# matteospanio/torchfx

Measured on AMD Instinct MI355X. Metric: Msamples/s/GPU (64-ch fused biquad→FIR→FFT-conv chain); % HBM roofline, higher is better.
Workload: dtype f64 (IIR) + f32 (FFT); f32 I/O

## Files before the change

### torchfx_amd/csrc/ols_kernels.h

```cpp
#pragma once
#include "common.h"
#include "epilogue.h"
#include "fftpk.h"

namespace tfx {

typedef float2 cpx;

__device__ __forceinline__ cpx cmul(cpx a, cpx b) { return make_float2(a.x * b.x - a.y * b.y, a.x * b.y + a.y * b.x); }
__device__ __forceinline__ cpx cmulc(cpx a, cpx b) { return make_float2(a.x * b.x + a.y * b.y, a.y * b.x - a.x * b.y); }
__device__ __forceinline__ cpx cadd(cpx a, cpx b) { return make_float2(a.x + b.x, a.y + b.y); }
__device__ __forceinline__ cpx csub(cpx a, cpx b) { return make_float2(a.x - b.x, a.y - b.y); }

template <bool INV>
__device__ __forceinline__ void dft4(cpx &a0, cpx &a1, cpx &a2, cpx &a3)
{
    const cpx s02 = cadd(a0, a2), d02 = csub(a0, a2), s13 = cadd(a1, a3), d13 = csub(a1, a3);
    const cpx id = INV ? make_float2(-d13.y, d13.x) : make_float2(d13.y, -d13.x);
    a0 = cadd(s02, s13);
    a2 = csub(s02, s13);
    a1 = cadd(d02, id);
    a3 = csub(d02, id);
}

__device__ __forceinline__ void wave_sync2()
{
    __builtin_amdgcn_fence(__ATOMIC_RELEASE, "wavefront");
    __builtin_amdgcn_wave_barrier();
    __builtin_amdgcn_fence(__ATOMIC_ACQUIRE, "wavefront");
}

struct OlsGeom {
    int64_t Tn;
    int64_t Tout;
    int64_t F;
    int64_t S;
    int64_t t0;
    int64_t pad_left;
    int64_t out_shift;
    int64_t nframes;
    const float *hist;
    int64_t H;
    float ep_gain;
    int ep_scale, ep_clamp, ep_stat;
    double *ep_partial;
    int64_t ep_row;
    int N2;
    int P2;
    int sh_on, sh_base;
    int *nf_flag;
    int *nf_pair;
    int nt;
};

constexpr int OLS_N1 = 256;
constexpr int OLS_CB = 32;

__device__ __forceinline__ int pad16(int p) { return p + (p >> 4); }
__device__ __forceinline__ int row_shift(const OlsGeom &g, int64_t c) { return g.sh_on ? (int)(((int64_t)g.sh_base + c * g.Tn) & 31) : 0; }


template <bool INV, int NBF, bool LEAN = false>
__device__ __forceinline__ void col_stages16(cpx (&v)[NBF][16], cpx *lds, const cpx *tw256, int col, int q)
{
    constexpr int QS = 16 / NBF;
    using pk::v2f;
    const v2f Wc = {0.92387953251128675613f, 0.38268343236508977173f}, Wr = {0.70710678118654752440f, 0.70710678118654752440f};
    v2f *L = (v2f *)lds;
    const v2f *TW = (const v2f *)tw256;
#pragma unroll
    for (int i = 0; i < NBF; ++i) {
        v2f u[16];
#pragma unroll
        for (int t = 0; t < 16; ++t) u[t] = __builtin_bit_cast(v2f, v[i][t]);
        pk::pk_dft16<INV>(u, Wc, Wr);
        const int j = q + QS * i;
#pragma unroll
        for (int k = 0; k < 16; ++k) L[(16 * j + k) * OLS_CB + col] = u[PK_DFT16_AT(k)];
    }
    __syncthreads();
#pragma unroll
    for (int i = 0; i < NBF; ++i) {
        const int j = q + QS * i;
        v2f d[16], w[16];
#pragma unroll
        for (int t = 0; t < 16; ++t) d[t] = L[(j + 16 * t) * OLS_CB + col];
        if (LEAN) {
#pragma unroll
            for (int b = 0; b < 4; ++b) {
#pragma unroll
                for (int t = 0; t < 4; ++t) if (4 * b + t > 0) w[t] = TW[((4 * b + t) * j) & 255];
                __builtin_amdgcn_sched_barrier(0);
#pragma unroll
                for (int t = 0; t < 4; ++t) if (4 * b + t > 0) d[4 * b + t] = pk::pk_cmul<INV>(d[4 * b + t], w[t]);
            }
        } else {
#pragma unroll
            for (int t = 1; t < 16; ++t) w[t] = TW[(t * j) & 255];
            __builtin_amdgcn_sched_barrier(0);
#pragma unroll
            for (int t = 1; t < 16; ++t) d[t] = pk::pk_cmul<INV>(d[t], w[t]);
        }
        pk::pk_dft16<INV>(d, Wc, Wr);
#pragma unroll
        for (int t = 0; t < 16; ++t) v[i][t] = __builtin_bit_cast(cpx, d[t]);
    }
}

template <int NBF>
__global__ void __launch_bounds__(512 / NBF, 2)
ols_col_fwd16_kernel(const float *__restrict__ x, cpx *__restrict__ T, const cpx *__restrict__ tw256g,
                     OlsGeom g, int64_t frame0)
{
    constexpr int QS = 16 / NBF;
    extern __shared__ __attribute__((aligned(16))) char smem[];
    cpx *lds = (cpx *)smem;
    cpx *tw256 = lds + OLS_N1 * OLS_CB;
    const int tid = threadIdx.x, col = tid & 31, q = tid >> 5;
    if (tid < 256) tw256[tid] = tw256g[tid];
    const int ncb = g.N2 / OLS_CB;
    const int64_t pair = blockIdx.x / ncb;
    const int cb = blockIdx.x % ncb;
    const int n2 = cb * OLS_CB + col;
    const int64_t fa = frame0 + 2 * pair, fb = fa + 1;
    const int64_t ca = fa / g.F, ia0 = g.t0 + (fa % g.F) * g.S - g.pad_left - row_shift(g, ca);
    const bool has_b = fb < g.nframes;
    const int64_t cb_ = has_b ? fb / g.F : 0, ib0 = has_b ? g.t0 + (fb % g.F) * g.S - g.pad_left - row_shift(g, cb_) : 0;
    const float *xa = x + ca * g.Tn, *xb = x + cb_ * g.Tn;
    cpx v[NBF][16];
    const int64_t span = (int64_t)OLS_N1 * g.N2;
    const bool inner = ia0 >= 0 && ia0 + span <= g.Tn && has_b && ib0 >= 0 && ib0 + span <= g.Tn;
    if (inner && (g.nt & 1)) {
#pragma unroll
        for (int i = 0; i < NBF; ++i)
#pragma unroll
            for (int t = 0; t < 16; ++t) {
                const int64_t n = (int64_t)(q + QS * i + 16 * t) * g.N2 + n2;
                v[i][t] = make_float2(__builtin_nontemporal_load(xa + ia0 + n), __builtin_nontemporal_load(xb + ib0 + n));
            }
    } else if (inner) {
#pragma unroll
        for (int i = 0; i < NBF; ++i)
#pragma unroll
            for (int t = 0; t < 16; ++t) {
                const int64_t n = (int64_t)(q + QS * i + 16 * t) * g.N2 + n2;
                v[i][t] = make_float2(xa[ia0 + n], xb[ib0 + n]);
            }
    } else {
#pragma unroll
        for (int i = 0; i < NBF; ++i)
#pragma unroll
            for (int t = 0; t < 16; ++t) {
                const int64_t n = (int64_t)(q + QS * i + 16 * t) * g.N2 + n2;
                const int64_t ia = ia0 + n, ib = ib0 + n;
                float re = (ia >= 0 && ia < g.Tn) ? xa[ia] : 0.0f;
                float im = (has_b && ib >= 0 && ib < g.Tn) ? xb[ib] : 0.0f;
                if (g.hist) {
                    if (ia < 0 && ia >= -g.H) re = g.hist[ca * g.H + g.H + ia];
                    if (has_b && ib < 0 && ib >= -g.H) im = g.hist[cb_ * g.H + g.H + ib];
                }
                v[i][t] = make_float2(re, im);
            }
    }
    if (has_b && ca != cb_ && g.nf_pair) {
        bool bad_a = false, bad_b = false;
#pragma unroll
        for (int i = 0; i < NBF; ++i)
#pragma unroll
            for (int t = 0; t < 16; ++t) {
                if (!(__builtin_fabsf(v[i][t].x) <= 3.4028234663852886e38f)) { v[i][t].x = 0.0f; bad_a = true; }
                if (!(__builtin_fabsf(v[i][t].y) <= 3.4028234663852886e38f)) { v[i][t].y = 0.0f; bad_b = true; }
            }
        if (bad_a) atomicOr(&g.nf_pair[ca], 2);
        if (bad_b) atomicOr(&g.nf_pair[cb_], 1);
    }
    __syncthreads();
    col_stages16<false, NBF>(v, lds, tw256, col, q);
    cpx *Tp = T + pair * ((int64_t)OLS_N1 * g.P2);
#pragma unroll
    for (int i = 0; i < NBF; ++i)
#pragma unroll
        for (int k = 0; k < 16; ++k)
            Tp[(int64_t)(q + QS * i + 16 * k) * g.P2 + n2] = v[i][PK_DFT16_AT(k)];
}

template <int NBF>
__global__ void __launch_bounds__(512 / NBF, 2)
ols_col_inv16_kernel(const cpx *__restrict__ T, float *__restrict__ y, const cpx *__restrict__ tw256g,
                     OlsGeom g, int64_t frame0)
{
    constexpr int QS = 16 / NBF;
    extern __shared__ __attribute__((aligned(16))) char smem[];
    cpx *lds = (cpx *)smem;
    cpx *tw256 = lds + OLS_N1 * OLS_CB;
    const int tid = threadIdx.x, col = tid & 31, q = tid >> 5;
    if (tid < 256) tw256[tid] = tw256g[tid];
    const int ncb = g.N2 / OLS_CB;
    const int64_t pair = blockIdx.x / ncb;
    const int cb = blockIdx.x % ncb;
    const int n2 = cb * OLS_CB + col;
    const cpx *Tp = T + pair * ((int64_t)OLS_N1 * g.P2);
    cpx v[NBF][16];
#pragma unroll
    for (int i = 0; i < NBF; ++i)
#pragma unroll
        for (int t = 0; t < 16; ++t) v[i][t] = Tp[(int64_t)(q + QS * i + 16 * t) * g.P2 + n2];
    __syncthreads();
    col_stages16<true, NBF>(v, lds, tw256, col, q);

    const int64_t fa = frame0 + 2 * pair, fb = fa + 1;
    const int64_t ca = fa / g.F, oa0 = g.t0 + (fa % g.F) * g.S;
    const bool has_b = fb < g.nframes;
    const int64_t cb_ = has_b ? fb / g.F : 0, ob0 = has_b ? g.t0 + (fb % g.F) * g.S : 0;
    float *ya = y + ca * g.Tout, *yb = y + cb_ * g.Tout;
    const int64_t sha = g.out_shift + row_shift(g, ca), shb = g.out_shift + row_shift(g, cb_);
    const bool epi = g.ep_scale | g.ep_clamp | (g.ep_stat >= 0);
    double acc_a = 0.0, acc_b = 0.0;
#pragma unroll
    for (int i = 0; i < NBF; ++i)
#pragma unroll
        for (int k = 0; k < 16; ++k) {
            const int64_t n = (int64_t)(q + QS * i + 16 * k) * g.N2 + n2;
            if (n < g.S) {
                cpx o = v[i][PK_DFT16_AT(k)];
                const int64_t oa = oa0 + n - sha, ob = ob0 + n - shb;
                const bool wa = oa >= 0 && oa < g.Tout, wb = has_b && ob >= 0 && ob < g.Tout;
                if (epi) {
                    if (g.ep_scale) { o.x *= g.ep_gain; o.y *= g.ep_gain; }
                    if (g.ep_clamp) { o.x = clamp_unit(o.x); o.y = clamp_unit(o.y); }
                    if (g.ep_stat >= 0) {
                        if (wa) acc_a = red_comb_rt(g.ep_stat, acc_a, red_elem_rt(g.ep_stat, (double)o.x));
                        if (wb) acc_b = red_comb_rt(g.ep_stat, acc_b, red_elem_rt(g.ep_stat, (double)o.y));
                    }
                }
                if (g.nt & 2) {
                    if (wa) __builtin_nontemporal_store(o.x, ya + oa);
                    if (wb) __builtin_nontemporal_store(o.y, yb + ob);
                } else {
                    if (wa) ya[oa] = o.x;
                    if (wb) yb[ob] = o.y;
                }
            }
        }
    if (g.ep_stat >= 0) {
        double *red = (double *)smem;
        __syncthreads();
#pragma unroll
        for (int off = 32; off >= 1; off >>= 1) {
            acc_a = red_comb_rt(g.ep_stat, acc_a, __shfl_xor(acc_a, off));
            acc_b = red_comb_rt(g.ep_stat, acc_b, __shfl_xor(acc_b, off));
        }
        const int nw = (int)(blockDim.x >> 6), w = tid >> 6;
        if ((tid & 63) == 0) { red[w] = acc_a; red[nw + w] = acc_b; }
        __syncthreads();
        if (tid == 0) {
            double ra = red[0], rb = red[nw];
            for (int u = 1; u < nw; ++u) { ra = red_comb_rt(g.ep_stat, ra, red[u]); rb = red_comb_rt(g.ep_stat, rb, red[nw + u]); }
            g.ep_partial[ca * g.ep_row + (fa % g.F) * ncb + cb] = ra;
            if (has_b) g.ep_partial[cb_ * g.ep_row + (fb % g.F) * ncb + cb] = rb;
        }
    }
}

__global__ void __launch_bounds__(256) ols_straddle_fix_kernel(float *__restrict__ y, OlsGeom g)
{
    const int64_t c = blockIdx.x;
    const int flag = g.nf_pair[c];
    if (!flag) return;
    const int64_t org = g.t0 - g.out_shift - row_shift(g, c);
    for (int e = 0; e < 2; ++e) {
        if (!(flag & (1 << e))) continue;
        const int64_t f = e ? g.F - 1 : 0;
        if (blockIdx.y == 0 && threadIdx.x == 0 && g.ep_stat >= 0) g.ep_partial[c * g.ep_row + f * (g.N2 / OLS_CB)] = __builtin_nan("");
        const int64_t lo = max((int64_t)0, org + f * g.S), hi = min(g.Tout, org + (f + 1) * g.S);
        for (int64_t t = lo + (int64_t)blockIdx.y * 256 + threadIdx.x; t < hi; t += (int64_t)gridDim.y * 256) y[c * g.Tout + t] = __builtin_nanf("");
    }
}

constexpr int SOSF_MAXK = 8;
constexpr int SOSF_K4W = 4;
constexpr int SOSF_CH = 16;
constexpr int SOSF_LS = 36;
constexpr size_t OLS_SHM_SOSF = (size_t)512 * SOSF_LS * sizeof(float) + 256 * sizeof(cpx);
struct SosFuse {
    double co[SOSF_MAXK][5];
    double *sections;
    int warm_blocks;
    int prio;
};

template <int KS, bool TAPS, bool UNIT>
__global__ void __launch_bounds__(512, ((KS <= SOSF_K4W && !TAPS) ? 4 : 2))
ols_col_fwd16_sos_kernel(const float *__restrict__ x, cpx *__restrict__ T, const cpx *__restrict__ tw256g,
                         OlsGeom g, int64_t frame0, SosFuse sf)
{
    extern __shared__ __attribute__((aligned(16))) char smem[];
    float *S = (float *)smem;
    cpx *lds = (cpx *)smem;
    cpx *tw256 = (cpx *)(smem + (size_t)512 * SOSF_LS * sizeof(float));
    const int tid = threadIdx.x;
    if (tid < 256) tw256[tid] = tw256g[tid];
    const int64_t pair = blockIdx.x;
    const int64_t fa = frame0 + 2 * pair, fb = fa + 1;
    const int64_t ca = fa / g.F, ia0 = g.t0 + (fa % g.F) * g.S - g.pad_left - row_shift(g, ca);
    const bool has_b = fb < g.nframes;
    const int64_t cb_ = has_b ? fb / g.F : 0, ib0 = has_b ? g.t0 + (fb % g.F) * g.S - g.pad_left - row_shift(g, cb_) : 0;
    const float *xa = x + ca * g.Tn, *xb = x + cb_ * g.Tn;
    const int nblk = g.N2 / OLS_CB;
    int64_t ta = ia0 - (int64_t)OLS_CB * sf.warm_blocks, tb = ib0 - (int64_t)OLS_CB * sf.warm_blocks;
    auto bound = [](int64_t v) { return (int)(v < -(int64_t)0x40000000 ? -(int64_t)0x40000000 : (v > (int64_t)0x40000000 ? (int64_t)0x40000000 : v)); };

    const bool mine_b = tid >= 256;
    const int rel_l = (tid & 255) * g.N2;
    const int own_lo = TAPS ? ((((mine_b ? fb : fa) % g.F) == 0 && g.t0 == 0) ? 0 : OLS_N1 * g.N2 - (int)g.S) : 0;
    double h1[KS + 1], h2[KS + 1];
#pragma unroll
    for (int s = 0; s <= KS; ++s) { h1[s] = 0.0; h2[s] = 0.0; }

    const int lrow = tid >> 3, lpart = tid & 7;
    const int rel_f = lrow * g.N2 + 4 * lpart;
    const int rstep = 64 * g.N2;
    float4 P[8];
    auto fetch = [&]() {
        const float *pa = xa + ta, *pb = xb + tb;
        const int lo_a = bound(-ta), hi_a = bound(g.Tn - ta), lo_b = bound(-tb), hi_b = has_b ? bound(g.Tn - tb) : lo_b;
        int rel = rel_f;
        asm volatile("" : "+v"(rel));
#pragma unroll
        for (int i = 0; i < 8; ++i) {
            const bool isb = i >= 4;
            const int r = rel + (i & 3) * rstep;
            const int lo = isb ? lo_b : lo_a, hi = isb ? hi_b : hi_a;
            float4 v = make_float4(0.f, 0.f, 0.f, 0.f);
            if (r >= lo && r + 4 <= hi) {
                const float *src = (isb ? pb : pa) + r;
                v = (g.nt & 1) ? ldg16_stream<float4>(src) : *(const float4 *)src;
            } else if (r + 4 > lo && r < hi) {
                const float *src = (isb ? pb : pa) + r;
                if (r >= lo) v.x = src[0];
                if (r + 1 >= lo && r + 1 < hi) v.y = src[1];
                if (r + 2 >= lo && r + 2 < hi) v.z = src[2];
                if (r + 3 < hi) v.w = src[3];
            }
            P[i] = v;
        }
        ta += OLS_CB; tb += OLS_CB;
    };
    fetch();
    cpx *Tp = T + pair * ((int64_t)OLS_N1 * g.P2);
    const int col = tid & 31, q = tid >> 5;
    for (int blk = -sf.warm_blocks; blk < nblk; ++blk) {
#pragma unroll
        for (int i = 0; i < 8; ++i) *(float4 *)&S[(lrow + 64 * i) * SOSF_LS + 4 * lpart] = P[i];
        int64_t tcur = (mine_b ? tb : ta) - OLS_CB;
        {
            const unsigned lo32 = (unsigned)__builtin_amdgcn_readfirstlane((int)(unsigned)(uint64_t)tcur);
            const unsigned hi32 = (unsigned)__builtin_amdgcn_readfirstlane((int)(unsigned)((uint64_t)tcur >> 32));
            tcur = (int64_t)(((uint64_t)hi32 << 32) | lo32);
        }
        const int last = (!mine_b || has_b) ? min(max(bound(g.Tn - tcur) - rel_l, 0), OLS_CB) : 0;
        int first = 0;
        if (TAPS) first = max(min(max(bound(-tcur) - rel_l, 0), OLS_CB), min(max(own_lo - (rel_l + OLS_CB * blk), 0), OLS_CB));
        if (blk + 1 < nblk) fetch();
        __syncthreads();
        if (sf.prio) __builtin_amdgcn_s_setprio(0);
#pragma unroll 1
        for (int j = 0; j < OLS_CB / SOSF_CH; ++j) {
            float u[SOSF_CH];
#pragma unroll
            for (int i = 0; i < SOSF_CH / 4; ++i) {
                const float4 w4 = *(const float4 *)&S[tid * SOSF_LS + SOSF_CH * j + 4 * i];
                u[4 * i] = w4.x; u[4 * i + 1] = w4.y; u[4 * i + 2] = w4.z; u[4 * i + 3] = w4.w;
            }
            const int lastj = last - SOSF_CH * j, firstj = first - SOSF_CH * j;
#pragma unroll
            for (int n = 0; n < SOSF_CH; ++n) {
                double v = (double)u[n];
#pragma unroll
                for (int s = 0; s < KS; ++s) {
                    double yn = UNIT ? __builtin_fma(sf.co[s][1], h1[s], v) : __builtin_fma(sf.co[s][1], h1[s], sf.co[s][0] * v);
                    yn = __builtin_fma(sf.co[s][2], h2[s], yn);
                    yn = __builtin_fma(sf.co[s][3], h1[s + 1], yn);
                    yn = __builtin_fma(sf.co[s][4], h2[s + 1], yn);
                    h2[s] = h1[s]; h1[s] = v;
                    v = yn;
                    if (TAPS) {
                        if (blk >= 0 && n >= firstj && n < lastj)
                            sf.sections[((int64_t)s * (g.nframes / g.F) + (mine_b ? cb_ : ca)) * g.Tn + tcur + rel_l + SOSF_CH * j + n] =
                                UNIT ? yn * sf.co[s][0] : yn;
                    }
                }
                h2[KS] = h1[KS]; h1[KS] = v;
                if (UNIT) v *= sf.co[KS - 1][0];
                u[n] = n < lastj ? (float)v : 0.0f;
            }
            if (blk >= 0) {
#pragma unroll
                for (int i = 0; i < SOSF_CH / 4; ++i)
                    *(float4 *)&S[tid * SOSF_LS + SOSF_CH * j + 4 * i] = make_float4(u[4 * i], u[4 * i + 1], u[4 * i + 2], u[4 * i + 3]);
                if (!(__builtin_fabs(h1[KS]) <= 1.7976931348623157e308)) {
#pragma unroll
                    for (int i = 0; i < SOSF_CH / 4; ++i)
                        *(float4 *)&S[tid * SOSF_LS + SOSF_CH * j + 4 * i] = make_float4(0.f, 0.f, 0.f, 0.f);
                }
            }
        }
        if (sf.prio) __builtin_amdgcn_s_setprio(3);
        if (blk < 0) { __syncthreads(); continue; }
        __syncthreads();
        cpx v[1][16];
#pragma unroll
        for (int t = 0; t < 16; ++t) v[0][t] = make_float2(S[(q + 16 * t) * SOSF_LS + col], S[(256 + q + 16 * t) * SOSF_LS + col]);
        __syncthreads();
        col_stages16<false, 1, true>(v, lds, tw256, col, q);
        char *Tb = (char *)(Tp + blk * OLS_CB);
        unsigned off = (unsigned)(q * g.P2 + col) * (unsigned)sizeof(cpx);
        asm volatile("" : "+v"(off));
        const unsigned ostep = 16u * (unsigned)g.P2 * (unsigned)sizeof(cpx);
#pragma unroll
        for (int k = 0; k < 16; ++k) { *(cpx *)(Tb + off) = v[0][PK_DFT16_AT(k)]; off += ostep; }
        __syncthreads();
    }
    {
        int *flag = (int *)smem;
        if (tid < 2) flag[tid] = 0;
        __syncthreads();
        const double e1 = h1[KS], e2 = h2[KS];
        if (!(__builtin_fabs(e1) <= 1.7976931348623157e308 && __builtin_fabs(e2) <= 1.7976931348623157e308)) flag[mine_b ? 1 : 0] = 1;
        __syncthreads();
        if (tid == 0) g.nf_flag[fa] = flag[0];
        if (tid == 1 && has_b) g.nf_flag[fb] = flag[1];
    }
}

__global__ void __launch_bounds__(256)
ols_sos_nonfinite_fix_kernel(float *__restrict__ y, double *__restrict__ sections, OlsGeom g, int warm_blocks, OlsGeom gt, int has_tail)
{
    __shared__ int s_first;
    __shared__ long long s_n;
    const int tid = threadIdx.x;
    const int64_t c = blockIdx.x;
    if (tid == 0) { s_first = 0x7fffffff; s_n = 0x7fffffffffffffffll; }
    __syncthreads();
    for (int64_t f = tid; f < g.F; f += 256)
        if (g.nf_flag[c * g.F + f]) atomicMin(&s_first, (int)f);
    __syncthreads();
    int64_t first = s_first;
    if (first == 0x7fffffff) {
        if (!has_tail || !gt.nf_flag[c]) return;
        g = gt;
        first = 0;
    }
    const int sh = row_shift(g, c);
    const float nanf_ = __builtin_nanf("");
    if (blockIdx.z == 0) {
        if (blockIdx.y == 0 && tid == 0 && g.ep_stat >= 0) g.ep_partial[c * g.ep_row + first * (g.N2 / OLS_CB)] = __builtin_nan("");
        const int64_t t0 = max((int64_t)0, g.t0 + first * g.S - g.out_shift - sh);
        const int64_t len = g.Tout - t0, per = (len + gridDim.y - 1) / gridDim.y;
        const int64_t lo = t0 + per * blockIdx.y, hi = min(g.Tout, lo + per);
        for (int64_t t = lo + tid; t < hi; t += 256) y[c * g.Tout + t] = nanf_;
        return;
    }
    if (!sections || blockIdx.y != 0) return;
    double *row = sections + ((int64_t)(blockIdx.z - 1) * (g.nframes / g.F) + c) * g.Tn;
    const int64_t start = max((int64_t)0, g.t0 + first * g.S - g.pad_left - sh - (int64_t)OLS_CB * warm_blocks);
    for (int64_t t0 = start; t0 < g.Tn; t0 += 4096) {
        int found = 0;
        for (int64_t t = t0 + tid; t < min(g.Tn, t0 + 4096); t += 256)
            if (!(__builtin_fabs(row[t]) <= 1.7976931348623157e308)) { atomicMin(&s_n, (long long)t); found = 1; break; }
        if (__syncthreads_or(found)) break;
    }
    const int64_t n = s_n;
    if (n == 0x7fffffffffffffffll) return;
    const double nan_ = __builtin_nan("");
    for (int64_t t = n + 1 + tid; t < g.Tn; t += 256) row[t] = nan_;
}

template <int L2, bool INV>
__device__ __forceinline__ void row_stages(cpx (&v)[(1 << (2 * L2)) / 256][4], cpx *lds, const cpx *twr, int lane)
{
    constexpr int N2 = 1 << (2 * L2), Q = N2 / 4, NB = Q / 64;
#pragma unroll
    for (int i = 0; i < NB; ++i) dft4<INV>(v[i][0], v[i][1], v[i][2], v[i][3]);
#pragma unroll
    for (int s = 1; s < L2; ++s) {
        const int Ns_prev = 1 << (2 * (s - 1));
        const int Ns = Ns_prev * 4;
#pragma unroll
        for (int i = 0; i < NB; ++i) {
            const int j = lane + 64 * i;
            const int j0 = (j / Ns_prev) * (4 * Ns_prev) + (j % Ns_prev);
#pragma unroll
            for (int r = 0; r < 4; ++r) lds[j0 + r * Ns_prev] = v[i][r];
        }
        wave_sync2();
#pragma unroll
        for (int i = 0; i < NB; ++i) {
            const int j = lane + 64 * i;
            const int k = j % Ns;
#pragma unroll
            for (int r = 0; r < 4; ++r) {
                cpx x = lds[j + Q * r];
                if (r > 0) {
                    const cpx w = twr[(r * k * (Q / Ns)) & (N2 - 1)];
                    x = INV ? cmulc(x, w) : cmul(x, w);
                }
                v[i][r] = x;
            }
            dft4<INV>(v[i][0], v[i][1], v[i][2], v[i][3]);
        }
        wave_sync2();
    }
}

template <int L2>
__global__ void __launch_bounds__(256)
ols_row_kernel(cpx *__restrict__ T, const cpx *__restrict__ Hp, const cpx *__restrict__ twrg,
               const cpx *__restrict__ tlo, const cpx *__restrict__ thi, int64_t nrows, int P2)
{
    constexpr int N2 = 1 << (2 * L2), Q = N2 / 4, NB = Q / 64;
    constexpr int64_t N = (int64_t)OLS_N1 * N2;
    extern __shared__ __attribute__((aligned(16))) char smem[];
    cpx *twr = (cpx *)smem;
    const int tid = threadIdx.x, lane = tid & 63, wave = tid >> 6;
    cpx *lds = twr + N2 + wave * N2;
    for (int i = tid; i < N2; i += 256) twr[i] = twrg[i];
    __syncthreads();
    const int64_t row = (int64_t)blockIdx.x * 4 + wave;
    if (row >= nrows) return;
    const int k1 = (int)(row % OLS_N1);
    cpx *base = T + row * P2;
    const cpx *hrow = Hp + (int64_t)k1 * N2;

    cpx v[NB][4], w[NB][4];
#pragma unroll
    for (int i = 0; i < NB; ++i) {
#pragma unroll
        for (int r = 0; r < 4; ++r) {
            const int n2 = lane + 64 * i + Q * r;
            const unsigned m = (unsigned)(((int64_t)k1 * n2) & (N - 1));
            w[i][r] = cmul(tlo[m & 511], thi[m >> 9]);
            v[i][r] = cmul(base[n2], w[i][r]);
        }
    }
    row_stages<L2, false>(v, lds, twr, lane);
#pragma unroll
    for (int i = 0; i < NB; ++i)
#pragma unroll
        for (int r = 0; r < 4; ++r) v[i][r] = cmul(v[i][r], hrow[lane + 64 * i + Q * r]);
    row_stages<L2, true>(v, lds, twr, lane);
#pragma unroll
    for (int i = 0; i < NB; ++i)
#pragma unroll
        for (int r = 0; r < 4; ++r) base[lane + 64 * i + Q * r] = cmulc(v[i][r], w[i][r]);
}

__global__ void __launch_bounds__(256, 3)
ols_row256pk_kernel(cpx *__restrict__ T, const cpx *__restrict__ Hp, const cpx *__restrict__ tw256g,
                    const cpx *__restrict__ tlo, const cpx *__restrict__ thi, int64_t nrows, int P2)
{
    using pk::v2f;
    extern __shared__ __attribute__((aligned(16))) char smem[];
    const int tid = threadIdx.x, lane = tid & 63, wave = tid >> 6, i = lane & 15, r = lane >> 4;
    v2f *L = (v2f *)smem + (wave * 4 + r) * 272;
    const v2f Wc = {0.92387953251128675613f, 0.38268343236508977173f}, Wr = {0.70710678118654752440f, 0.70710678118654752440f};
    v2f tw[16];
#pragma unroll
    for (int k = 1; k < 16; ++k) tw[k] = ((const v2f *)tw256g)[(i * k) & 255];
    for (int64_t row0 = ((int64_t)blockIdx.x * 4 + wave) * 4; row0 < nrows; row0 += (int64_t)gridDim.x * 16) {
        const int64_t row = row0 + r;
        const bool live = row < nrows;
        const int k1 = (int)((live ? row : 0) % OLS_N1);
        v2f *base = (v2f *)(T + (live ? row : 0) * P2);
        const v2f *hrow = (const v2f *)(Hp + (int64_t)k1 * 256);
        v2f w[16];
        {
            const unsigned ma = (unsigned)(k1 * i), mb = (unsigned)(16 * k1);
            const v2f wl = pk::pk_cmul<false>(((const v2f *)tlo)[ma & 511], ((const v2f *)thi)[ma >> 9]);
            v2f u[16];
            u[1] = pk::pk_cmul<false>(((const v2f *)tlo)[mb & 511], ((const v2f *)thi)[mb >> 9]);
            u[2] = pk::pk_cmul<false>(u[1], u[1]);
            u[3] = pk::pk_cmul<false>(u[2], u[1]);
            u[4] = pk::pk_cmul<false>(u[2], u[2]);
            u[5] = pk::pk_cmul<false>(u[4], u[1]);
            u[6] = pk::pk_cmul<false>(u[4], u[2]);
            u[7] = pk::pk_cmul<false>(u[4], u[3]);
            u[8] = pk::pk_cmul<false>(u[4], u[4]);
#pragma unroll
            for (int t = 9; t < 16; ++t) u[t] = pk::pk_cmul<false>(u[8], u[t - 8]);
            w[0] = wl;
#pragma unroll
            for (int t = 1; t < 16; ++t) w[t] = pk::pk_cmul<false>(wl, u[t]);
        }
        v2f v[16];
#pragma unroll
        for (int t = 0; t < 16; ++t) v[t] = live ? base[i + 16 * t] : v2f{0.f, 0.f};
        __builtin_amdgcn_sched_barrier(0);
#pragma unroll
        for (int t = 0; t < 16; ++t) v[t] = pk::pk_cmul<false>(v[t], w[t]);
        pk::pk_dft16<false>(v, Wc, Wr);
        L[17 * i] = v[PK_DFT16_AT(0)];
#pragma unroll
        for (int k = 1; k < 16; ++k) L[17 * i + k] = pk::pk_cmul<false>(v[PK_DFT16_AT(k)], tw[k]);
        wave_sync2();
#pragma unroll
        for (int t = 0; t < 16; ++t) v[t] = L[17 * t + i];
        wave_sync2();
        pk::pk_dft16<false>(v, Wc, Wr);
        v2f h[16];
#pragma unroll
        for (int k = 0; k < 16; ++k) h[k] = hrow[i + 16 * k];
        __builtin_amdgcn_sched_barrier(0);
        v2f z[16];
#pragma unroll
        for (int k = 0; k < 16; ++k) z[k] = pk::pk_cmul<false>(v[PK_DFT16_AT(k)], h[k]);
        pk::pk_dft16<true>(z, Wc, Wr);
        L[17 * i] = z[PK_DFT16_AT(0)];
#pragma unroll
        for (int k = 1; k < 16; ++k) L[17 * i + k] = pk::pk_cmul<true>(z[PK_DFT16_AT(k)], tw[k]);
        wave_sync2();
#pragma unroll
        for (int t = 0; t < 16; ++t) z[t] = L[17 * t + i];
        wave_sync2();
        pk::pk_dft16<true>(z, Wc, Wr);
        if (live) {
#pragma unroll
            for (int t = 0; t < 16; ++t) base[i + 16 * t] = pk::pk_cmul<true>(z[PK_DFT16_AT(t)], w[t]);
        }
    }
}

template <bool INV>
__device__ __forceinline__ void row_fft1024_pk(pk::v2f (&v)[16], pk::v2f *lds, const pk::v2f *twr, int lane, pk::v2f Wc, pk::v2f Wr)
{
    using pk::v2f;
    pk::pk_dft16<INV>(v, Wc, Wr);
#pragma unroll
    for (int k = 0; k < 16; ++k) lds[pad16(16 * lane + k)] = v[PK_DFT16_AT(k)];
    wave_sync2();
    const int kb = lane & 15;
    {
        v2f d[16], w[16];
#pragma unroll
        for (int t = 0; t < 16; ++t) d[t] = lds[pad16(lane + 64 * t)];
#pragma unroll
        for (int t = 1; t < 16; ++t) w[t] = twr[(4 * t * kb) & 1023];
        __builtin_amdgcn_sched_barrier(0);
        v[0] = d[0];
#pragma unroll
        for (int t = 1; t < 16; ++t) v[t] = pk::pk_cmul<INV>(d[t], w[t]);
    }
    wave_sync2();
    pk::pk_dft16<INV>(v, Wc, Wr);
    const int j0 = (lane >> 4) * 256 + kb;
#pragma unroll
    for (int k = 0; k < 16; ++k) lds[pad16(j0 + 16 * k)] = v[PK_DFT16_AT(k)];
    wave_sync2();
    {
        v2f d[16], w[16];
#pragma unroll
        for (int i = 0; i < 4; ++i)
#pragma unroll
            for (int r = 0; r < 4; ++r) {
                d[i + 4 * r] = lds[pad16(lane + 64 * i + 256 * r)];
                if (r > 0) w[i + 4 * r] = twr[(r * (lane + 64 * i)) & 1023];
            }
        __builtin_amdgcn_sched_barrier(0);
#pragma unroll
        for (int i = 0; i < 4; ++i) {
#pragma unroll
            for (int r = 1; r < 4; ++r) d[i + 4 * r] = pk::pk_cmul<INV>(d[i + 4 * r], w[i + 4 * r]);
            pk::pk_dft4<INV, false>(d[i], d[i + 4], d[i + 8], d[i + 12]);
        }
#pragma unroll
        for (int t = 0; t < 16; ++t) v[t] = d[t];
    }
    wave_sync2();
}

__global__ void __launch_bounds__(256, 3)
ols_row1024_kernel(cpx *__restrict__ T, const cpx *__restrict__ Hp, const cpx *__restrict__ twrg,
                   const cpx *__restrict__ tlo, const cpx *__restrict__ thi, const cpx *__restrict__ tu,
                   int64_t nrows, int64_t Nmask, int P2)
{
    constexpr int N2 = 1024, LDSROW = N2 + N2 / 16;
    extern __shared__ __attribute__((aligned(16))) char smem[];
    cpx *twr = (cpx *)smem;
    const int tid = threadIdx.x, lane = tid & 63;
    const int wave = __builtin_amdgcn_readfirstlane(tid >> 6);
    cpx *lds = twr + N2 + wave * LDSROW;
    for (int i = tid; i < N2; i += 256) twr[i] = twrg[i];
    __syncthreads();
    const int64_t row = (int64_t)blockIdx.x * 4 + wave;
    if (row >= nrows) return;
    const int k1 = (int)(row % OLS_N1);
    cpx *base = T + row * P2;
    const cpx *hrow = Hp + (int64_t)k1 * N2;
    typedef const float __attribute__((address_space(4))) *cfp;
    const cfp tuc = (cfp)(uintptr_t)tu;

    const unsigned ml = (unsigned)(k1 * lane);
    const cpx wl = cmul(tlo[ml & 511], thi[ml >> 9]);
    using pk::v2f;
    const v2f Wc = {0.92387953251128675613f, 0.38268343236508977173f}, Wr = {0.70710678118654752440f, 0.70710678118654752440f};
    v2f u[16], h[16];
#pragma unroll
    for (int t = 0; t < 16; ++t) h[t] = ((const v2f *)base)[lane + 64 * t];
    __builtin_amdgcn_sched_barrier(0);
#pragma unroll
    for (int t = 0; t < 16; ++t) {
        const unsigned iu = 2u * ((unsigned)(k1 * t) & (unsigned)(Nmask >> 6));
        const cpx w = cmul(wl, make_float2(tuc[iu], tuc[iu + 1]));
        u[t] = pk::pk_cmul<false>(h[t], __builtin_bit_cast(v2f, w));
    }
    row_fft1024_pk<false>(u, (v2f *)lds, (const v2f *)twr, lane, Wc, Wr);
    __builtin_amdgcn_sched_barrier(0);
#pragma unroll
    for (int t = 0; t < 16; ++t) h[t] = ((const v2f *)hrow)[lane + 64 * t];
    __builtin_amdgcn_sched_barrier(0);
#pragma unroll
    for (int t = 0; t < 16; ++t) u[t] = pk::pk_cmul<false>(u[t], h[t]);
    __builtin_amdgcn_sched_barrier(0);
    row_fft1024_pk<true>(u, (v2f *)lds, (const v2f *)twr, lane, Wc, Wr);
    float wlx = wl.x, wly = wl.y;
    asm volatile("" : "+v"(wlx), "+v"(wly));
    const cpx wl2 = make_float2(wlx, wly);
#pragma unroll
    for (int t = 0; t < 16; ++t) {
        const unsigned iu = 2u * ((unsigned)(k1 * t) & (unsigned)(Nmask >> 6));
        const cpx w = cmul(wl2, make_float2(tuc[iu], tuc[iu + 1]));
        ((v2f *)base)[lane + 64 * t] = pk::pk_cmul<true>(u[t], __builtin_bit_cast(v2f, w));
    }
}

template <int MAP>
__global__ void __launch_bounds__(256, 4)
ols_row4096_kernel(cpx *__restrict__ T, const cpx *__restrict__ Hp, const cpx *__restrict__ tw256g,
                   const cpx *__restrict__ t4log, const cpx *__restrict__ t4hig,
                   const cpx *__restrict__ tlo, const cpx *__restrict__ thi, const cpx *__restrict__ tu,
                   int64_t Nmask, int P2, int64_t npairs)
{
    constexpr int N2 = 4096;
    extern __shared__ __attribute__((aligned(16))) char smem[];
    cpx *lds = (cpx *)smem;
    cpx *twB = lds + N2 + N2 / 16;
    cpx *twA = twB + 256;
    const int j = threadIdx.x;
    twB[j] = tw256g[((j >> 4) * (j & 15)) & 255];
    twA[j] = t4log[j];
    typedef const float __attribute__((address_space(4))) *cfp;
    const cfp tuc = (cfp)(uintptr_t)tu;
    const unsigned umask = (unsigned)(Nmask >> 8);
    int k1;
    int64_t p;
    if (MAP == 0) {
        k1 = (int)(blockIdx.x % OLS_N1);
        p = blockIdx.x / OLS_N1;
    } else {
        const unsigned xcd = blockIdx.x & 7u, m = blockIdx.x >> 3;
        k1 = (int)((m / (unsigned)npairs) * 8u + xcd);
        p = m % (unsigned)npairs;
    }
    __syncthreads();
    const cpx *hrow = Hp + (int64_t)k1 * N2;
    const unsigned ml = (unsigned)(k1 * j);
    const cpx wl = cmul(tlo[ml & 511], thi[ml >> 9]);
    cpx *base = T + (p * OLS_N1 + k1) * P2;
    using pk::v2f;
    const v2f Wc = {0.92387953251128675613f, 0.38268343236508977173f}, Wr = {0.70710678118654752440f, 0.70710678118654752440f};
    v2f u[16], h[16];
#pragma unroll
    for (int t = 0; t < 16; ++t) h[t] = ((const v2f *)base)[j + 256 * t];
    __builtin_amdgcn_sched_barrier(0);
#pragma unroll
    for (int t = 0; t < 16; ++t) {
        const unsigned iu = 2u * ((unsigned)(k1 * t) & umask);
        const cpx w = cmul(wl, make_float2(tuc[iu], tuc[iu + 1]));
        u[t] = pk::pk_cmul<false>(h[t], __builtin_bit_cast(v2f, w));
    }
    pk::fft4096_pk<false>(u, (v2f *)lds, (const v2f *)twB, (const v2f *)twA, j, Wc, Wr);
    __builtin_amdgcn_sched_barrier(0);
#pragma unroll
    for (int t = 0; t < 16; ++t) h[t] = ((const v2f *)hrow)[j + 256 * t];
    __builtin_amdgcn_sched_barrier(0);
#pragma unroll
    for (int t = 0; t < 16; ++t) u[t] = pk::pk_cmul<false>(u[t], h[t]);
    __builtin_amdgcn_sched_barrier(0);
    pk::fft4096_pk<true>(u, (v2f *)lds, (const v2f *)twB, (const v2f *)twA, j, Wc, Wr);
    float wlx = wl.x, wly = wl.y;
    asm volatile("" : "+v"(wlx), "+v"(wly));
    const cpx wl2 = make_float2(wlx, wly);
#pragma unroll
    for (int t = 0; t < 16; ++t) {
        const unsigned iu = 2u * ((unsigned)(k1 * t) & umask);
        const cpx w = cmul(wl2, make_float2(tuc[iu], tuc[iu + 1]));
        ((v2f *)base)[j + 256 * t] = pk::pk_cmul<true>(u[t], __builtin_bit_cast(v2f, w));
    }
}


__device__ __forceinline__ int row8192_at(int k2)
{
    const int h = k2 & 1, m = k2 >> 1, t = m >> 8, jj = m & 255;
    return ((h * 8 + (t >> 1)) * 256 + jj) * 2 + (t & 1);
}
inline int row8192_at_host(int k2)
{
    const int h = k2 & 1, m = k2 >> 1, t = m >> 8, jj = m & 255;
    return ((h * 8 + (t >> 1)) * 256 + jj) * 2 + (t & 1);
}

template <int MAP>
__global__ void __launch_bounds__(256, 4)
ols_row8192_kernel(cpx *__restrict__ T, const cpx *__restrict__ Hp, const cpx *__restrict__ tw256g,
                   const cpx *__restrict__ t4log, const cpx *__restrict__ tlo, const cpx *__restrict__ thi,
                   const cpx *__restrict__ tu, const cpx *__restrict__ w8kg, int64_t Nmask, int P2, int64_t npairs)
{
    using pk::v2f;
    using pk::v4f;
    constexpr int N2 = 8192;
    extern __shared__ __attribute__((aligned(16))) char smem[];
    cpx *lds = (cpx *)smem;
    cpx *twBc = lds + 4096 + 256;
    cpx *twAc = twBc + 256;
    const int j = threadIdx.x;
    twBc[j] = tw256g[((j >> 4) * (j & 15)) & 255];
    twAc[j] = t4log[j];
    typedef const float __attribute__((address_space(4))) *cfp;
    const cfp tuc = (cfp)(uintptr_t)tu;
    const unsigned umask = (unsigned)(Nmask >> 8);
    int k1;
    int64_t p;
    if (MAP == 0) {
        k1 = (int)(blockIdx.x % OLS_N1);
        p = blockIdx.x / OLS_N1;
    } else {
        const unsigned xcd = blockIdx.x & 7u, m = blockIdx.x >> 3;
        k1 = (int)((m / (unsigned)npairs) * 8u + xcd);
        p = m % (unsigned)npairs;
    }
    const v2f wj = ((const v2f *)w8kg)[j];
    __syncthreads();
    const v2f *twB = (const v2f *)twBc, *twA = (const v2f *)twAc;
    const v4f *Hq = (const v4f *)(Hp + (int64_t)k1 * N2);
    const unsigned ml = (unsigned)(k1 * j);
    const cpx wl = cmul(tlo[ml & 511], thi[ml >> 9]);
    cpx *base = T + (p * OLS_N1 + k1) * P2;
    const v2f Wc = {0.92387953251128675613f, 0.38268343236508977173f}, Wr = {0.70710678118654752440f, 0.70710678118654752440f};
    char *rowb = (char *)base;
    unsigned roff = (unsigned)j * (unsigned)sizeof(cpx);
    asm volatile("" : "+v"(roff));
    v2f a[16], b[16];
#pragma unroll
    for (int half = 0; half < 2; ++half) {
        v2f lo[8], hi[8];
#pragma unroll
        for (int u = 0; u < 8; ++u) {
            const int t = 8 * half + u;
            lo[u] = *(const v2f *)(rowb + (roff + 2048u * (unsigned)t));
            hi[u] = *(const v2f *)(rowb + (roff + 2048u * (unsigned)(t + 16)));
        }
        __builtin_amdgcn_sched_barrier(0);
#pragma unroll
        for (int u = 0; u < 8; ++u) {
            const int t = 8 * half + u;
            const unsigned i0 = 2u * ((unsigned)(k1 * t) & umask), i1 = 2u * ((unsigned)(k1 * (t + 16)) & umask);
            const cpx w0 = cmul(wl, make_float2(tuc[i0], tuc[i0 + 1])), w1 = cmul(wl, make_float2(tuc[i1], tuc[i1 + 1]));
            const v2f l = pk::pk_cmul<false>(lo[u], __builtin_bit_cast(v2f, w0)), h = pk::pk_cmul<false>(hi[u], __builtin_bit_cast(v2f, w1));
            const v2f w = t ? pk::pk_cmul<false>(wj, twB[16 * t + 8]) : wj;
            a[t] = l + h;
            b[t] = pk::pk_cmul<false>(l - h, w);
        }
        __builtin_amdgcn_sched_barrier(0);
    }
    pk::fft4096_pk<false>(a, (v2f *)lds, twB, twA, j, Wc, Wr);
    {
        v4f q[8];
#pragma unroll
        for (int m = 0; m < 8; ++m) q[m] = Hq[m * 256 + j];
        __builtin_amdgcn_sched_barrier(0);
#pragma unroll
        for (int m = 0; m < 8; ++m) {
            a[2 * m] = pk::pk_cmul<false>(a[2 * m], v2f{q[m].x, q[m].y});
            a[2 * m + 1] = pk::pk_cmul<false>(a[2 * m + 1], v2f{q[m].z, q[m].w});
        }
    }
    pk::fft4096_pk<false>(b, (v2f *)lds, twB, twA, j, Wc, Wr);
    {
        v4f q[8];
#pragma unroll
        for (int m = 0; m < 8; ++m) q[m] = Hq[(8 + m) * 256 + j];
        __builtin_amdgcn_sched_barrier(0);
#pragma unroll
        for (int m = 0; m < 8; ++m) {
            b[2 * m] = pk::pk_cmul<false>(b[2 * m], v2f{q[m].x, q[m].y});
            b[2 * m + 1] = pk::pk_cmul<false>(b[2 * m + 1], v2f{q[m].z, q[m].w});
        }
    }
    pk::fft4096_pk<true>(a, (v2f *)lds, twB, twA, j, Wc, Wr);
    pk::fft4096_pk<true>(b, (v2f *)lds, twB, twA, j, Wc, Wr);
    float wlx = wl.x, wly = wl.y;
    asm volatile("" : "+v"(wlx), "+v"(wly));
    const cpx wl2 = make_float2(wlx, wly);
    v2f wj2 = wj;
    asm volatile("" : "+v"(wj2));
    unsigned roff2 = (unsigned)j * (unsigned)sizeof(cpx);
    asm volatile("" : "+v"(roff2));
#pragma unroll
    for (int t = 0; t < 16; ++t) {
        const v2f w = t ? pk::pk_cmul<false>(wj2, twB[16 * t + 8]) : wj2;
        const v2f bw = pk::pk_cmul<true>(b[t], w);
        const unsigned i0 = 2u * ((unsigned)(k1 * t) & umask), i1 = 2u * ((unsigned)(k1 * (t + 16)) & umask);
        const cpx w0 = cmul(wl2, make_float2(tuc[i0], tuc[i0 + 1])), w1 = cmul(wl2, make_float2(tuc[i1], tuc[i1 + 1]));
        *(v2f *)(rowb + (roff2 + 2048u * (unsigned)t)) = pk::pk_cmul<true>(a[t] + bw, __builtin_bit_cast(v2f, w0));
        *(v2f *)(rowb + (roff2 + 2048u * (unsigned)(t + 16))) = pk::pk_cmul<true>(a[t] - bw, __builtin_bit_cast(v2f, w1));
    }
}

__global__ void __launch_bounds__(256, 4)
ols_rowspec4096_kernel(cpx *__restrict__ T, const cpx *__restrict__ tw256g, const cpx *__restrict__ t4log,
                       const cpx *__restrict__ tlo, const cpx *__restrict__ thi, const cpx *__restrict__ tu,
                       int64_t Nmask, int P2, float inv_n)
{
    using pk::v2f;
    extern __shared__ __attribute__((aligned(16))) char smem[];
    cpx *lds = (cpx *)smem;
    cpx *twB = lds + 4096 + 256;
    cpx *twA = twB + 256;
    const int j = threadIdx.x;
    twB[j] = tw256g[((j >> 4) * (j & 15)) & 255];
    twA[j] = t4log[j];
    typedef const float __attribute__((address_space(4))) *cfp;
    const cfp tuc = (cfp)(uintptr_t)tu;
    const unsigned umask = (unsigned)(Nmask >> 8);
    const int k1 = (int)blockIdx.x;
    __syncthreads();
    const unsigned ml = (unsigned)(k1 * j);
    const cpx wl = cmul(tlo[ml & 511], thi[ml >> 9]);
    cpx *base = T + (int64_t)k1 * P2;
    const v2f Wc = {0.92387953251128675613f, 0.38268343236508977173f}, Wr = {0.70710678118654752440f, 0.70710678118654752440f};
    v2f u[16];
#pragma unroll
    for (int t = 0; t < 16; ++t) {
        const unsigned iu = 2u * ((unsigned)(k1 * t) & umask);
        const cpx w = cmul(wl, make_float2(tuc[iu], tuc[iu + 1]));
        u[t] = pk::pk_cmul<false>(((const v2f *)base)[j + 256 * t], __builtin_bit_cast(v2f, w));
    }
    pk::fft4096_pk<false>(u, (v2f *)lds, (const v2f *)twB, (const v2f *)twA, j, Wc, Wr);
#pragma unroll
    for (int t = 0; t < 16; ++t) base[j + 256 * t] = make_float2(u[t].x * inv_n, -u[t].y * inv_n);
}

__global__ void __launch_bounds__(256, 4)
ols_rowspec8192_kernel(cpx *__restrict__ T, const cpx *__restrict__ tw256g, const cpx *__restrict__ t4log,
                       const cpx *__restrict__ tlo, const cpx *__restrict__ thi, const cpx *__restrict__ tu,
                       const cpx *__restrict__ w8kg, int64_t Nmask, int P2, float inv_n)
{
    using pk::v2f;
    extern __shared__ __attribute__((aligned(16))) char smem[];
    cpx *lds = (cpx *)smem;
    cpx *twBc = lds + 4096 + 256;
    cpx *twAc = twBc + 256;
    const int j = threadIdx.x;
    twBc[j] = tw256g[((j >> 4) * (j & 15)) & 255];
    twAc[j] = t4log[j];
    typedef const float __attribute__((address_space(4))) *cfp;
    const cfp tuc = (cfp)(uintptr_t)tu;
    const unsigned umask = (unsigned)(Nmask >> 8);
    const int k1 = (int)blockIdx.x;
    const v2f wj = ((const v2f *)w8kg)[j];
    __syncthreads();
    const v2f *twB = (const v2f *)twBc, *twA = (const v2f *)twAc;
    const unsigned ml = (unsigned)(k1 * j);
    const cpx wl = cmul(tlo[ml & 511], thi[ml >> 9]);
    cpx *base = T + (int64_t)k1 * P2;
    const v2f Wc = {0.92387953251128675613f, 0.38268343236508977173f}, Wr = {0.70710678118654752440f, 0.70710678118654752440f};
    v2f a[16], b[16];
#pragma unroll
    for (int t = 0; t < 16; ++t) {
        const unsigned i0 = 2u * ((unsigned)(k1 * t) & umask), i1 = 2u * ((unsigned)(k1 * (t + 16)) & umask);
        const cpx w0 = cmul(wl, make_float2(tuc[i0], tuc[i0 + 1])), w1 = cmul(wl, make_float2(tuc[i1], tuc[i1 + 1]));
        const v2f l = pk::pk_cmul<false>(((const v2f *)base)[j + 256 * t], __builtin_bit_cast(v2f, w0));
        const v2f h = pk::pk_cmul<false>(((const v2f *)base)[j + 256 * (t + 16)], __builtin_bit_cast(v2f, w1));
        const v2f w = t ? pk::pk_cmul<false>(wj, twB[16 * t + 8]) : wj;
        a[t] = l + h;
        b[t] = pk::pk_cmul<false>(l - h, w);
    }
    pk::fft4096_pk<false>(a, (v2f *)lds, twB, twA, j, Wc, Wr);
    pk::fft4096_pk<false>(b, (v2f *)lds, twB, twA, j, Wc, Wr);
#pragma unroll
    for (int t = 0; t < 16; ++t) {
        base[((0 * 8 + (t >> 1)) * 256 + j) * 2 + (t & 1)] = make_float2(a[t].x * inv_n, -a[t].y * inv_n);
        base[((1 * 8 + (t >> 1)) * 256 + j) * 2 + (t & 1)] = make_float2(b[t].x * inv_n, -b[t].y * inv_n);
    }
}

}
```

Baseline: 202,000.

## Specialize fused SOS recursion into warm, interior and edge paths with buffer loads

Splits the fused biquad recursion loop into three compile-time modes. Warm-up blocks skip all output handling, interior blocks skip the per-sample bound masks and write results as they go, and edge blocks keep the original masked logic. When both frames lie fully inside the signal, the input is fetched with unmasked raw buffer loads instead of per-element bounds checks. The twiddle table is also stored in LDS as a [16][16] table indexed directly, which removes the multiply-and-mask address math in the lean DFT. The cost is more code paths, plus a static_assert that ties the lean path to NBF==1.

```diff
diff --git a/torchfx_amd/csrc/ols_kernels.h b/torchfx_amd/csrc/ols_kernels.h
--- a/torchfx_amd/csrc/ols_kernels.h
+++ b/torchfx_amd/csrc/ols_kernels.h
@@ -86,10 +86,11 @@
 #pragma unroll
         for (int t = 0; t < 16; ++t) d[t] = L[(j + 16 * t) * OLS_CB + col];
         if (LEAN) {
+            static_assert(!LEAN || NBF == 1, "the lean form reads a [16][16] table: j = q < 16");
 #pragma unroll
             for (int b = 0; b < 4; ++b) {
 #pragma unroll
-                for (int t = 0; t < 4; ++t) if (4 * b + t > 0) w[t] = TW[((4 * b + t) * j) & 255];
+                for (int t = 0; t < 4; ++t) if (4 * b + t > 0) w[t] = TW[16 * j + 4 * b + t];
                 __builtin_amdgcn_sched_barrier(0);
 #pragma unroll
                 for (int t = 0; t < 4; ++t) if (4 * b + t > 0) d[4 * b + t] = pk::pk_cmul<INV>(d[4 * b + t], w[t]);
@@ -280,6 +281,7 @@
 constexpr int SOSF_MAXK = 8;
 constexpr int SOSF_K4W = 4;
 constexpr int SOSF_CH = 16;
+constexpr int SOSF_EDGE = 0, SOSF_INNER = 1, SOSF_WARM = 2;
 constexpr int SOSF_LS = 36;
 constexpr size_t OLS_SHM_SOSF = (size_t)512 * SOSF_LS * sizeof(float) + 256 * sizeof(cpx);
 struct SosFuse {
@@ -299,7 +301,7 @@
     cpx *lds = (cpx *)smem;
     cpx *tw256 = (cpx *)(smem + (size_t)512 * SOSF_LS * sizeof(float));
     const int tid = threadIdx.x;
-    if (tid < 256) tw256[tid] = tw256g[tid];
+    if (tid < 256) tw256[tid] = tw256g[(tid >> 4) * (tid & 15)];
     const int64_t pair = blockIdx.x;
     const int64_t fa = frame0 + 2 * pair, fb = fa + 1;
     const int64_t ca = fa / g.F, ia0 = g.t0 + (fa % g.F) * g.S - g.pad_left - row_shift(g, ca);
@@ -311,20 +313,23 @@
     auto bound = [](int64_t v) { return (int)(v < -(int64_t)0x40000000 ? -(int64_t)0x40000000 : (v > (int64_t)0x40000000 ? (int64_t)0x40000000 : v)); };
 
     const bool mine_b = tid >= 256;
-    const int rel_l = (tid & 255) * g.N2;
     const int own_lo = TAPS ? ((((mine_b ? fb : fa) % g.F) == 0 && g.t0 == 0) ? 0 : OLS_N1 * g.N2 - (int)g.S) : 0;
     double h1[KS + 1], h2[KS + 1];
 #pragma unroll
     for (int s = 0; s <= KS; ++s) { h1[s] = 0.0; h2[s] = 0.0; }
 
     const int lrow = tid >> 3, lpart = tid & 7;
-    const int rel_f = lrow * g.N2 + 4 * lpart;
+    auto rel_f = [&]() {
+        int t = tid;
+        asm volatile("" : "+v"(t));
+        return (t >> 3) * g.N2 + 4 * (t & 7);
+    };
     const int rstep = 64 * g.N2;
     float4 P[8];
     auto fetch = [&]() {
         const float *pa = xa + ta, *pb = xb + tb;
         const int lo_a = bound(-ta), hi_a = bound(g.Tn - ta), lo_b = bound(-tb), hi_b = has_b ? bound(g.Tn - tb) : lo_b;
-        int rel = rel_f;
+        int rel = rel_f();
         asm volatile("" : "+v"(rel));
 #pragma unroll
         for (int i = 0; i < 8; ++i) {
@@ -346,7 +351,30 @@
         }
         ta += OLS_CB; tb += OLS_CB;
     };
-    fetch();
+    const int64_t in_hi = g.Tn - ((int64_t)(OLS_N1 - 1) * g.N2 + OLS_CB);
+    auto interior = [&](int64_t t) { return ((int)((uint64_t)t >> 32) | (int)(((uint64_t)in_hi - (uint64_t)t) >> 32)) >= 0; };
+    const bool nt_ld = (g.nt & 1) != 0;
+    auto fetch_interior = [&]() {
+        const int extent = (int)((OLS_N1 - 1) * g.N2 + OLS_CB) * (int)sizeof(float);
+        const __amdgpu_buffer_rsrc_t ra = __builtin_amdgcn_make_buffer_rsrc((void *)(xa + ta), 0, extent, 0x00020000);
+        const __amdgpu_buffer_rsrc_t rb = __builtin_amdgcn_make_buffer_rsrc((void *)(xb + tb), 0, extent, 0x00020000);
+        const int off = rel_f() * (int)sizeof(float), step = rstep * (int)sizeof(float);
+        if (nt_ld) {
+#pragma unroll
+            for (int i = 0; i < 8; ++i)
+                P[i] = __builtin_bit_cast(float4, __builtin_amdgcn_raw_buffer_load_b128(i >= 4 ? rb : ra, off, (i & 3) * step, 2));
+        } else {
+#pragma unroll
+            for (int i = 0; i < 8; ++i)
+                P[i] = __builtin_bit_cast(float4, __builtin_amdgcn_raw_buffer_load_b128(i >= 4 ? rb : ra, off, (i & 3) * step, 0));
+        }
+        ta += OLS_CB; tb += OLS_CB;
+    };
+    auto fetch_next = [&]() {
+        if (!TAPS && has_b && interior(ta) && interior(tb)) fetch_interior();
+        else fetch();
+    };
+    fetch_next();
     cpx *Tp = T + pair * ((int64_t)OLS_N1 * g.P2);
     const int col = tid & 31, q = tid >> 5;
     for (int blk = -sf.warm_blocks; blk < nblk; ++blk) {
@@ -358,53 +386,70 @@
             const unsigned hi32 = (unsigned)__builtin_amdgcn_readfirstlane((int)(unsigned)((uint64_t)tcur >> 32));
             tcur = (int64_t)(((uint64_t)hi32 << 32) | lo32);
         }
-        const int last = (!mine_b || has_b) ? min(max(bound(g.Tn - tcur) - rel_l, 0), OLS_CB) : 0;
-        int first = 0;
-        if (TAPS) first = max(min(max(bound(-tcur) - rel_l, 0), OLS_CB), min(max(own_lo - (rel_l + OLS_CB * blk), 0), OLS_CB));
-        if (blk + 1 < nblk) fetch();
+        const bool keep_all = !TAPS && (__builtin_amdgcn_readfirstlane(tid) < 256 || has_b) && interior(tcur);
+        if (blk + 1 < nblk) fetch_next();
         __syncthreads();
         if (sf.prio) __builtin_amdgcn_s_setprio(0);
+        auto recur = [&](auto mode_) {
+            constexpr int MODE = decltype(mode_)::value;
+            int last = OLS_CB, first = 0, rel_l = 0;
+            if (MODE == SOSF_EDGE) {
+                int row = tid & 255;
+                asm volatile("" : "+v"(row));
+                rel_l = row * g.N2;
+                last = (!mine_b || has_b) ? min(max(bound(g.Tn - tcur) - rel_l, 0), OLS_CB) : 0;
+                if (TAPS) first = max(min(max(bound(-tcur) - rel_l, 0), OLS_CB), min(max(own_lo - (rel_l + OLS_CB * blk), 0), OLS_CB));
+            }
 #pragma unroll 1
-        for (int j = 0; j < OLS_CB / SOSF_CH; ++j) {
-            float u[SOSF_CH];
-#pragma unroll
-            for (int i = 0; i < SOSF_CH / 4; ++i) {
-                const float4 w4 = *(const float4 *)&S[tid * SOSF_LS + SOSF_CH * j + 4 * i];
-                u[4 * i] = w4.x; u[4 * i + 1] = w4.y; u[4 * i + 2] = w4.z; u[4 * i + 3] = w4.w;
-            }
-            const int lastj = last - SOSF_CH * j, firstj = first - SOSF_CH * j;
-#pragma unroll
-            for (int n = 0; n < SOSF_CH; ++n) {
-                double v = (double)u[n];
-#pragma unroll
-                for (int s = 0; s < KS; ++s) {
-                    double yn = UNIT ? __builtin_fma(sf.co[s][1], h1[s], v) : __builtin_fma(sf.co[s][1], h1[s], sf.co[s][0] * v);
-                    yn = __builtin_fma(sf.co[s][2], h2[s], yn);
-                    yn = __builtin_fma(sf.co[s][3], h1[s + 1], yn);
-                    yn = __builtin_fma(sf.co[s][4], h2[s + 1], yn);
-                    h2[s] = h1[s]; h1[s] = v;
-                    v = yn;
-                    if (TAPS) {
-                        if (blk >= 0 && n >= firstj && n < lastj)
-                            sf.sections[((int64_t)s * (g.nframes / g.F) + (mine_b ? cb_ : ca)) * g.Tn + tcur + rel_l + SOSF_CH * j + n] =
-                                UNIT ? yn * sf.co[s][0] : yn;
+            for (int j = 0; j < OLS_CB / SOSF_CH; ++j) {
+                float u[SOSF_CH];
+#pragma unroll
+                for (int i = 0; i < SOSF_CH / 4; ++i) {
+                    const float4 w4 = *(const float4 *)&S[tid * SOSF_LS + SOSF_CH * j + 4 * i];
+                    u[4 * i] = w4.x; u[4 * i + 1] = w4.y; u[4 * i + 2] = w4.z; u[4 * i + 3] = w4.w;
+                }
+                const int lastj = last - SOSF_CH * j, firstj = first - SOSF_CH * j;
+#pragma unroll
+                for (int n = 0; n < SOSF_CH; ++n) {
+                    double v = (double)u[n];
+#pragma unroll
+                    for (int s = 0; s < KS; ++s) {
+                        double yn = UNIT ? __builtin_fma(sf.co[s][1], h1[s], v) : __builtin_fma(sf.co[s][1], h1[s], sf.co[s][0] * v);
+                        yn = __builtin_fma(sf.co[s][2], h2[s], yn);
+                        yn = __builtin_fma(sf.co[s][3], h1[s + 1], yn);
+                        yn = __builtin_fma(sf.co[s][4], h2[s + 1], yn);
+                        h2[s] = h1[s]; h1[s] = v;
+                        v = yn;
+                        if (TAPS && MODE == SOSF_EDGE) {
+                            if (blk >= 0 && n >= firstj && n < lastj)
+                                sf.sections[((int64_t)s * (g.nframes / g.F) + (mine_b ? cb_ : ca)) * g.Tn + tcur + rel_l + SOSF_CH * j + n] =
+                                    UNIT ? yn * sf.co[s][0] : yn;
+                        }
+                    }
+                    h2[KS] = h1[KS]; h1[KS] = v;
+                    if (MODE == SOSF_WARM) continue;
+                    if (UNIT) v *= sf.co[KS - 1][0];
+                    u[n] = (MODE == SOSF_INNER || n < lastj) ? (float)v : 0.0f;
+                    if (MODE == SOSF_INNER && (n & 3) == 3)
+                        *(float4 *)&S[tid * SOSF_LS + SOSF_CH * j + n - 3] = make_float4(u[n - 3], u[n - 2], u[n - 1], u[n]);
+                }
+                if (MODE != SOSF_WARM && blk >= 0) {
+                    if (MODE == SOSF_EDGE) {
+#pragma unroll
+                        for (int i = 0; i < SOSF_CH / 4; ++i)
+                            *(float4 *)&S[tid * SOSF_LS + SOSF_CH * j + 4 * i] = make_float4(u[4 * i], u[4 * i + 1], u[4 * i + 2], u[4 * i + 3]);
+                    }
+                    if (!(__builtin_fabs(h1[KS]) <= 1.7976931348623157e308)) {
+#pragma unroll
+                        for (int i = 0; i < SOSF_CH / 4; ++i)
+                            *(float4 *)&S[tid * SOSF_LS + SOSF_CH * j + 4 * i] = make_float4(0.f, 0.f, 0.f, 0.f);
                     }
                 }
-                h2[KS] = h1[KS]; h1[KS] = v;
-                if (UNIT) v *= sf.co[KS - 1][0];
-                u[n] = n < lastj ? (float)v : 0.0f;
             }
-            if (blk >= 0) {
-#pragma unroll
-                for (int i = 0; i < SOSF_CH / 4; ++i)
-                    *(float4 *)&S[tid * SOSF_LS + SOSF_CH * j + 4 * i] = make_float4(u[4 * i], u[4 * i + 1], u[4 * i + 2], u[4 * i + 3]);
-                if (!(__builtin_fabs(h1[KS]) <= 1.7976931348623157e308)) {
-#pragma unroll
-                    for (int i = 0; i < SOSF_CH / 4; ++i)
-                        *(float4 *)&S[tid * SOSF_LS + SOSF_CH * j + 4 * i] = make_float4(0.f, 0.f, 0.f, 0.f);
-                }
-            }
-        }
+        };
+        if (!TAPS && blk < 0) recur(std::integral_constant<int, SOSF_WARM>());
+        else if (keep_all) recur(std::integral_constant<int, SOSF_INNER>());
+        else recur(std::integral_constant<int, SOSF_EDGE>());
         if (sf.prio) __builtin_amdgcn_s_setprio(3);
         if (blk < 0) { __syncthreads(); continue; }
         __syncthreads();
```

After: 201,800 (median of 2 runs). About the same (-0.1%).
